# vocdoni/gnark-crypto-primitives

Measured on AMD Instinct MI355X. Metric: proofs/sec, Arbo-160 Poseidon SMT-verifier circuit, Groth16/BN254, higher is better.
Workload: dtype u32x8 Montgomery (254-bit integer)

## Files before the change

### gnark_crypto_primitives_amd/csrc/api.hip

```cpp
#include <algorithm>

#include "zkmi_internal.h"
#include "comb_plan.h"
#include "ff29.h"
#include "ec29.h"

using namespace zk;

namespace zk {

void sync_side_streams(zkmi_ctx* ctx) {
  for (hipStream_t q : {ctx->stream2, ctx->stream3, ctx->stream4})
    if (q) hipStreamSynchronize(q);
}

int ensure_scratch(zkmi_ctx* ctx, DevBuf& s, size_t bytes, void** out) {
  if (s.bytes < bytes) {
    if (s.p) {
      hipStreamSynchronize(ctx->stream);
      sync_side_streams(ctx);
      hipFree(s.p);
      s.p = nullptr;
      s.bytes = 0;
    }
// ... 334 lines not shown
  hipSetDevice(ctx->device);
  hipStreamSynchronize(ctx->stream);
  sync_side_streams(ctx);
  for (auto& st : ctx->sets) {
    if (st.ev0) hipEventDestroy(st.ev0);
    if (st.ev1) hipEventDestroy(st.ev1);
    for (auto& e : st.evq)
      if (e) hipEventDestroy(e);
    for (auto& e : st.eva)
      if (e) hipEventDestroy(e);
    if (st.tail_ev) hipEventDestroy(st.tail_ev);
    for (auto& p : st.msm_ev) {
      if (p[0]) hipEventDestroy(p[0]);
      if (p[1]) hipEventDestroy(p[1]);
    }
  }
  hipStreamDestroy(ctx->stream2);
  hipStreamDestroy(ctx->stream3);
  hipStreamDestroy(ctx->stream4);
  for (auto& p : ctx->plans) free_plan(p);
  for (auto& st : ctx->sets)
    for (DevBuf* b : {&st.slots, &st.a, &st.b, &st.c, &st.misc, &st.sums, &st.commit})
      if (b->p) hipFree(b->p);
  for (DevBuf* b : {&ctx->ntt_tmp, &ctx->build_tmp, &ctx->msm_digits, &ctx->msm_sint,
                    &ctx->msm_rowvar, &ctx->msm_part[0], &ctx->msm_part[1], &ctx->side_part2, &ctx->side_part3})
    if (b->p) hipFree(b->p);
  witness_ring_free(ctx);
  for (auto& e : ctx->ev)
    if (e) hipEventDestroy(e);
  for (auto& e : ctx->part_ev)
    if (e) hipEventDestroy(e);
  for (auto& e : ctx->acc_ev)
    if (e) hipEventDestroy(e);
  for (auto& e : ctx->dig_ev)
    if (e) hipEventDestroy(e);
  hipStreamDestroy(ctx->stream);
  delete ctx;
}

const char* zkmi_last_error(zkmi_ctx* ctx) { return ctx ? ctx->err.c_str() : "null context"; }

int zkmi_sync(zkmi_ctx* ctx) {
  ZK_HIP(hipStreamSynchronize(ctx->stream));
  return ZKMI_OK;
}

void* zkmi_stream(zkmi_ctx* ctx) { return (void*)ctx->stream; }
// ... 159 lines not shown
      if (plan.comb <= 8) return rc;
      plan = plan_comb(plan.comb - 1, plan.comb_signed != 0);
    } else if (plan.shared) {
      if (plan.bits[0] <= 4) return rc;
      plan = plan_shared(plan.bits[0] - 1);
    } else {
      if (plan.W >= 64) return rc;
      plan = plan_with_windows(plan.W + 1);
    }
  }
}

static bool window_bits_ok(int wb) {
  return wb == 0 || (wb >= 2 && wb <= 16) || (wb >= 104 && wb <= 116) ||
         (wb >= 202 && wb <= 220) || (wb >= 303 && wb <= 321);
}
static WinPlan plan_explicit(int wb) {
  return wb >= 300   ? plan_comb(wb - 300, true)
         : wb >= 200 ? plan_comb(wb - 200, false)
         : wb >= 100 ? plan_shared(wb - 100)
                     : plan_uniform(wb);
}
static double prove_working_set_bytes(uint32_t log_n, size_t n_slots, size_t n_in, size_t max_batch,
                                      size_t n_msm_max, size_t n_commitments) {
  const size_t Bp = round_up(max_batch ? max_batch : 1024, 64);
  const size_t n = (size_t)1 << log_n;
  const SetBytes sb = prove_set_bytes(n_slots, n, n_in, Bp, Bp);
  const double set = (double)(sb.slots + 3 * sb.abc + sb.misc + sums_bytes(Bp) +
                              commit_buffer_bytes(n_commitments, Bp));
  const double digits = 254.0 * (double)((n_msm_max + 15) / 16) * Bp * 4;
  const double sint = (double)n_msm_max * Bp * 32;
  const double partials = 2 * (21.0 * 254 * Bp * 256 + 256.0 * (double)((n_msm_max + 15) / 16) * 4);
  const double ring = 3.0 * std::max(68e6, (double)n_in * 32 * 64);
  return 2 * set + (double)n * Bp * 32 + digits + sint + partials + ring + 2e9 + 1e9;
}
static double free_hbm_bytes() {
  size_t free_b = 0, total_b = 0;
  if (hipMemGetInfo(&free_b, &total_b) != hipSuccess) free_b = (size_t)64 << 30;
  return (double)free_b;
}
static double usable_table_bytes_standalone(size_t n) {
  const double ws = (double)n * 1024 * 32 * 2 + 254.0 * ((n + 15) / 16) * 1024 * 4 +
                    21.0 * 254 * 1024 * 256 + 3e9;
  const double usable = free_hbm_bytes() - ws;
  return usable > 0 ? usable : 0.0;
}

int zkmi_msm_bases_load(zkmi_ctx* ctx, int group, const void* bases, size_t n, int window_bits,
                        zkmi_msm_bases** out) {
  return zkmi_msm_bases_load_image(ctx, group, bases, n, window_bits, 0, out);
}

int zkmi_msm_bases_load_image(zkmi_ctx* ctx, int group, const void* bases, size_t n,
                              int window_bits, int image, zkmi_msm_bases** out) {
  ZK_HIP(hipSetDevice(ctx->device));
  if (!out) return ZKMI_ERR_ARG;
  if (image != 0 && image != 1) {
// ... 301 lines not shown
  const uint32_t n_kb = fold.folded ? (uint32_t)fold.k_wire.size() : d->n_k;
  const uint32_t n_zb = fold.folded ? n_z + 1 : n_z;
  auto* pk = new zkmi_pk();
  pk->log_n = d->log_n;
  pk->n_wires = d->n_wires;
  pk->n_a = d->n_a;
  pk->n_b = d->n_b;
  pk->n_k = n_kb;
  pk->n_z = n_zb;
  pk->folded = fold.folded;
  pk->fold_n_constraints = fold.folded ? d->fold_r1cs->n_constraints : 0;
  pk->max_batch = d->max_batch ? d->max_batch : 1024;
  int rc;
  if ((rc = commit_keys_load(ctx, d, pk))) {
    zkmi_pk_free(ctx, pk);
    return rc;
  }
  const bool auto1 = d->window_bits_g1 == 0, auto2 = d->window_bits_g2 == 0;
  const size_t n1 = (size_t)d->n_a + d->n_b + n_kb + n_zb;
  const size_t n_msm_max = std::max(std::max((size_t)d->n_a, (size_t)d->n_b),
                                    std::max((size_t)n_kb, (size_t)n_zb));
  const size_t n_slots = d->n_slots_hint ? d->n_slots_hint : (size_t)d->n_wires + d->n_wires / 20;
  const double ws = prove_working_set_bytes(d->log_n, n_slots, d->n_wires, pk->max_batch, n_msm_max,
                                            pk->commits.size());
  double usable = free_hbm_bytes() - ws;
  if (usable < 0) usable = 0;
  if (d->table_budget_bytes && (double)d->table_budget_bytes < usable)
    usable = (double)d->table_budget_bytes;
  int sc1 = 0, sc2 = 0;
  plan_shared_for_budget(n1, d->n_b, 0.98 * usable, &sc1, &sc2);
  WinPlan p1 = auto1 ? plan_windows_for_budget(n1, 1, 0.64 * usable)
                     : plan_explicit((int)d->window_bits_g1);
  WinPlan p2 = auto2 ? plan_windows_for_budget(d->n_b, 2, 0.34 * usable)
                     : plan_explicit((int)d->window_bits_g2);
  if (auto1 && sc1 && plan_shared(sc1).W < p1.W) p1 = plan_shared(sc1);
  if (auto2 && sc2 && plan_shared(sc2).W < p2.W) p2 = plan_shared(sc2);
  WinPlan pm[COMB_PLAN_MSMS] = {p1, p1, p1, p1, p2};
  if (n1 >= 4096) {
    const size_t nm[COMB_PLAN_MSMS] = {auto1 ? d->n_a : 0u, auto1 ? d->n_b : 0u, auto1 ? n_kb : 0u,
                                       auto1 ? n_zb : 0u, auto2 ? d->n_b : 0u};
    const CombPlan eq = comb_plan_equal5(nm, 0.98 * usable, d->sparse_witness == 0);
    const CombPlan cp = comb_plan_search(nm, 0.98 * usable, d->sparse_witness == 0);
    for (int i = 0; i < COMB_PLAN_MSMS; i++) {
      const bool g2 = comb_msm_is_g2(i);
      if ((g2 ? auto2 : auto1) && (double)COMB_W / eq.k[i] < (double)(g2 ? p2 : p1).W)
        pm[i] = plan_comb(cp.k[i], cp.sg[i]);
    }
// ... 15 lines not shown
  bool relax[COMB_PLAN_MSMS] = {auto1, auto1, auto1, auto1, auto2};
  if (msm_window_bits)
    for (int i = 0; i < COMB_PLAN_MSMS; i++) {
      pm[i] = plan_explicit((int)msm_window_bits[i]);
      relax[i] = false;
    }
  auto load = [&](int group, const void* pts, size_t n, const WinPlan& plan, bool relax,
                  zkmi_msm_bases** out, int image) -> int {
    Staged sb(ctx);
    int r = sb.in(pts, n * (group == 1 ? 64 : 128));
    if (r) return r;
    r = bases_load_plan(ctx, group, sb.dev, n, plan, relax, out, image);
    if (!r) (*out)->chunk_factor = d->msm_chunk_factor;
    return r;
  };
  if ((rc = upload_u32(ctx, wa.data(), d->n_a, &pk->a_wire)) ||
      (rc = upload_u32(ctx, wb.data(), d->n_b, &pk->b_wire)) ||
      (rc = upload_u32(ctx, fold.folded ? fold.k_wire.data() : wk.data(), n_kb, &pk->k_wire)) ||
      (rc = load(1, d->g1_a, d->n_a, pm[COMB_MSM_A], relax[COMB_MSM_A], &pk->A, MSM_IMAGE_F)) ||
      (rc = load(1, d->g1_b, d->n_b, pm[COMB_MSM_B1], relax[COMB_MSM_B1], &pk->B1, MSM_IMAGE_F)) ||
      (rc = load(1, fold.folded ? (const void*)fold.k.data() : d->g1_k, n_kb, pm[COMB_MSM_K],
                 relax[COMB_MSM_K], &pk->K, MSM_IMAGE_F)) ||
      (rc = load(1, fold.folded ? (const void*)fold.e.data() : d->g1_z, n_zb, pm[COMB_MSM_Z],
                 relax[COMB_MSM_Z], &pk->Z, MSM_IMAGE_STD)) ||
      (rc = load(2, d->g2_b, d->n_b, pm[COMB_MSM_B2], relax[COMB_MSM_B2], &pk->B2, MSM_IMAGE_F))) {
    zkmi_pk_free(ctx, pk);
    return rc;
  }
  {
    const uint32_t idx[3] = {0, 1, 2};
    if ((rc = upload_u32(ctx, idx, 3, &pk->idx3)) ||
        (rc = zkmi_msm_bases_load(ctx, 1, d->g1_delta, 1, 8, &pk->D1)) ||
        (rc = zkmi_msm_bases_load(ctx, 2, d->g2_delta, 1, 8, &pk->D2))) {
      zkmi_pk_free(ctx, pk);
      return rc;
    }
    pk->D1->side = pk->D2->side = 2;
  }
  hipMemcpy(&pk->alpha, d->g1_alpha, 64, hipMemcpyDefault);
  hipMemcpy(&pk->beta1, d->g1_beta, 64, hipMemcpyDefault);
  hipMemcpy(&pk->delta1, d->g1_delta, 64, hipMemcpyDefault);
  hipMemcpy(&pk->beta2, d->g2_beta, 128, hipMemcpyDefault);
  hipMemcpy(&pk->delta2, d->g2_delta, 128, hipMemcpyDefault);
  *out = pk;
  return ZKMI_OK;
}

// ... 195 lines not shown
    if (!rc) rc = solve_rows(ctx, cs, slots, a, b, c, st, Bp, begin, cs->n_rows);
    if (!rc) rc = commit_finish_submit(ctx, S);
  }
  return prove_set_end(ctx, main, rc);
}

static int enqueue_heavy(zkmi_ctx* ctx, int si) {
  zkmi_ctx::ProveSet& S = ctx->sets[si];
  const zkmi_pk* pk = S.pk;
  const bool fd = S.f_domain;
  const size_t Bp = S.Bp, batch = S.batch, n = (size_t)1 << pk->log_n;
  NttPlan* plan;
  int rc = get_plan(ctx, (int)pk->log_n, &plan);
  if (rc) return rc;
  void* t0;
  if ((rc = ensure_scratch(ctx, ctx->ntt_tmp, n * Bp * 32, &t0))) return rc;
  SumsView v(S.sums.p, Bp);
  Fr* rs_bi = (Fr*)S.rs;
  Fr* slots = (Fr*)S.slots.p;
  ZK_HIP(hipStreamWaitEvent(ctx->stream, S.ev1, 0));
  hipEventRecord(S.evq[0], ctx->stream);
  Fr* h;
  if ((rc = pk->folded ? compute_ab_coset_bi(ctx, plan, (Fr*)S.a.p, (Fr*)S.b.p, (Fr*)t0, Bp,
                                             S.n_constraints, &h, fd)
                       : compute_h_bi(ctx, plan, (Fr*)S.a.p, (Fr*)S.b.p, (Fr*)S.c.p, (Fr*)t0, Bp,
                                      S.n_constraints, &h, fd)))
    return rc;
  hipEventRecord(S.evq[1], ctx->stream);
  S.msm_ev_used = 0;
  ctx->msm_ev_set = si;
  const bool d1 = pk->Z->plan.shared || pk->Z->plan.comb;
  const bool d2 = pk->B2->plan.shared || pk->B2->plan.comb;
  hipStream_t q3 = ctx->stream3, q4 = ctx->stream4;
  uint8_t* rv = nullptr;
  if (pk->A->plan.comb || pk->B2->plan.comb) {
    void* p;
    if ((rc = ensure_scratch(ctx, ctx->msm_rowvar, pk->n_wires, &p)) ||
        (rc = msm_rows_vary(ctx, slots, pk->n_wires, Bp, batch, (uint8_t*)p))) {
      ctx->msm_ev_set = -1;
      return rc;
    }
    rv = (uint8_t*)p;
  }
  if ((rc = msm_run(ctx, pk->A, slots, pk->a_wire, Bp, batch, v.sA, fd, d1 ? v.w1[0] : nullptr, q4,
                    rv)) ||
      (rc = msm_run(ctx, pk->B1, slots, pk->b_wire, Bp, batch, v.sB1, fd, d1 ? v.w1[1] : nullptr, q4,
                    rv)) ||
      (rc = msm_run(ctx, pk->K, slots, pk->k_wire, Bp, batch, v.sK, fd, d1 ? v.w1[2] : nullptr, q4,
                    rv)) ||
      (rc = msm_run(ctx, pk->Z, h, nullptr, Bp, batch, v.sZ, false, d1 ? v.w1[3] : nullptr, q4,
                    nullptr, true))) {
    ctx->msm_ev_set = -1;
    return rc;
  }
  hipEventRecord(S.evq[2], ctx->stream);
  rc = msm_run(ctx, pk->B2, slots, pk->b_wire, Bp, batch, v.sB2, fd, d2 ? v.w2 : nullptr, q4, rv);
  ctx->msm_ev_set = -1;
  if (rc) return rc;
  hipEventRecord(S.evq[3], ctx->stream);
  ZK_HIP(hipEventRecord(S.tail_ev, q4));
  {
    hipStream_t main_stream = ctx->stream;
    ZK_HIP(hipStreamWaitEvent(q3, S.ev1, 0));
    ctx->stream = q3;
    hipLaunchKernelGGL(rs_prep_kernel, dim3((unsigned)(Bp / 64)), dim3(64), 0, q3, rs_bi, Bp);
    (void)((rc = msm_run(ctx, pk->D1, rs_bi, pk->idx3 + 0, Bp, batch, v.tR)) ||
           (rc = msm_run(ctx, pk->D1, rs_bi, pk->idx3 + 1, Bp, batch, v.tS)) ||
           (rc = msm_run(ctx, pk->D1, rs_bi, pk->idx3 + 2, Bp, batch, v.tNRS)) ||
           (rc = msm_run(ctx, pk->D2, rs_bi, pk->idx3 + 1, Bp, batch, v.tS2)));
    ctx->stream = main_stream;
    if (rc) return rc;
  }
  if ((rc = commit_pok(ctx, S))) return rc;
  hipEventRecord(S.evq[4], ctx->stream);
// ... 109 lines not shown
```

### gnark_crypto_primitives_amd/csrc/ntt.hip

```cpp
#include <cstdlib>

#include "zkmi_internal.h"
#include "ff29.h"
#if defined(__HIP_DEVICE_COMPILE__)
#include "ff29_asm.h"
#endif

namespace zk {

__device__ __forceinline__ uint32_t pass_row(uint32_t hi, uint32_t q, uint32_t lo, int s0, int K) {
  return (hi << (s0 + K)) | (q << s0) | lo;
}

__device__ __forceinline__ uint32_t bitrev32(uint32_t x, int bits) {
  return __brev(x) >> (32 - bits);
}

__device__ __forceinline__ Fr29 ld29(const Fr* base, size_t row, size_t b, size_t Bp) {
  const Fr v = bi_ld(base, row, b, Bp);
  return unpack29<Fr29Params>(v.v);
}
__device__ __forceinline__ Fr29 ldz29(const Fr* base, size_t row, size_t b, size_t Bp) {
  const Fr v = bi_ld(base, row, b, Bp);
  return unpack_lazy<Fr29Params>(v.v);
}
__device__ __forceinline__ Fr29 ldc29(const Fr* tab, uint32_t i) {
  return unpack29<Fr29Params>(tab[i].v);
}

template <class T> __device__ __forceinline__ T ld_tw(const Fr* tw, uint32_t i);
template <> __device__ __forceinline__ Fr ld_tw<Fr>(const Fr* tw, uint32_t i) { return tw[i]; }
template <> __device__ __forceinline__ Fr29 ld_tw<Fr29>(const Fr* tw, uint32_t i) {
  return ldc29(tw, i);
}
__device__ __forceinline__ Fr tmul(const Fr& a, const Fr& tw) { return mul(a, tw); }
#if defined(__HIP_DEVICE_COMPILE__)
__device__ __forceinline__ Fr29 tmul(const Fr29& a, const Fr29& tw) { return mul_asm_s(a, tw); }
#else
ZK_HD Fr29 tmul(const Fr29& a, const Fr29& tw) { return mul(a, tw); }
#endif

template <int J0, int NJ, int LQ = J0, bool FROM0 = false, class T, int M>
__device__ __forceinline__ void butterflies(T (&x)[M], uint32_t qb, int log_n, int s0, uint32_t lo,
                                            const Fr* __restrict__ tw) {
#pragma unroll
  for (int j = J0; j < J0 + NJ; j++) {
    const int s = (FROM0 ? 0 : s0) + j, jj = j - LQ;
// ... 126 lines not shown
#pragma unroll
  for (int i = 0; i < 4; i++) {
    const uint32_t q = w + 4 * i;
    const uint4 l = xch[(q * 2 + 0) * 64 + lane], h = xch[(q * 2 + 1) * 64 + lane];
    x[i].v[0] = l.x; x[i].v[1] = l.y; x[i].v[2] = l.z; x[i].v[3] = l.w;
    x[i].v[4] = h.x; x[i].v[5] = h.y; x[i].v[6] = h.z; x[i].v[7] = h.w;
  }
  butterflies<2, 2, 2, FIRST>(x, w, log_n, s0, lo, tw);
#pragma unroll
  for (int i = 0; i < 4; i++)
    store_scaled<LAST>(dst, pass_row(hi, w + 4 * i, lo, s0, 4), b, Bp, x[i], post, post_uniform,
                       use_uniform);
}

template <bool FIRST, bool LAST>
__global__ __launch_bounds__(256) void ntt_pass4_lds29(const Fr* __restrict__ src,
                                                       Fr* __restrict__ dst, size_t Bp, int log_n,
                                                       int s0, const Fr* __restrict__ tw,
                                                       const Fr* __restrict__ pre, int in_std,
                                                       const Fr* __restrict__ post,
                                                       Fr post_uniform, int use_uniform,
                                                       uint32_t n_valid,
                                                       const Fr* __restrict__ sub_after,
                                                       const Fr* __restrict__ times) {
  __shared__ int32_t xch[16 * 9 * 64];
  const uint32_t lane = threadIdx.x;
  const size_t b = (size_t)blockIdx.x * 64 + lane;
  const uint32_t w = __builtin_amdgcn_readfirstlane(threadIdx.y);
  const uint32_t g = blockIdx.y;
  const uint32_t lo = g & ((1u << s0) - 1u);
  const uint32_t hi = g >> s0;
  Fr29 x[4];
#pragma unroll
  for (int i = 0; i < 4; i++) {
    const uint32_t row = pass_row(hi, 4 * w + i, lo, s0, 4);
    x[i] = FIRST ? first_load29(src, row, b, Bp, log_n, n_valid, pre, in_std)
                 : ldz29(dst, row, b, Bp);
  }
  butterflies<0, 2, 0, FIRST>(x, 4 * w, log_n, s0, lo, tw);
  exchange29(xch, x, w, w, lane);
  butterflies<2, 2, 2, FIRST>(x, w, log_n, s0, lo, tw);
#pragma unroll
  for (int i = 0; i < 4; i++) {
    const uint32_t row = pass_row(hi, w + 4 * i, lo, s0, 4);
    Fr out;
    if (LAST && (use_uniform || post)) {
      const Fr29 k = use_uniform ? unpack29<Fr29Params>(post_uniform.v) : ldc29(post, row);
      Fr29 v = norm(x[i]);
      if (times) v = mul(v, ldz29(times, row, b, Bp));
      pack_canonical<Fr29Params>(out.v, mul(v, k));
      if (sub_after) out = sub(out, bi_ld(sub_after, row, b, Bp));
    } else {
      pack_lazy<Fr29Params>(out.v, wred(x[i]));
    }
    bi_st(dst, row, b, Bp, out);
  }
}

template <int K>
__global__ __launch_bounds__(256) void ntt_mid29(Fr* __restrict__ dst, size_t Bp, int log_n, int s0,
                                                 const Fr* __restrict__ tw) {
  const size_t b = (size_t)blockIdx.x * 64 + threadIdx.x;
  const uint32_t g =
      __builtin_amdgcn_readfirstlane(blockIdx.y * blockDim.y + threadIdx.y);
  const uint32_t lo = g & ((1u << s0) - 1u);
  const uint32_t hi = g >> s0;
  constexpr int M = 1 << K;
  Fr29 x[M];
#pragma unroll
  for (int i = 0; i < M; i++) x[i] = ldz29(dst, pass_row(hi, i, lo, s0, K), b, Bp);
  butterflies<0, (K < 2 ? K : 2)>(x, 0, log_n, s0, lo, tw);
  if constexpr (K == 3) {
#pragma unroll
    for (int i = 0; i < M; i++) x[i] = norm(x[i]);
    butterflies<2, 1, 0>(x, 0, log_n, s0, lo, tw);
  }
#pragma unroll
  for (int i = 0; i < M; i++) {
    Fr out;
    pack_lazy<Fr29Params>(out.v, wred(x[i]));
    bi_st(dst, pass_row(hi, i, lo, s0, K), b, Bp, out);
  }
}

template <bool PRODUCT>
__global__ __launch_bounds__(256) void ntt_fused29(const Fr* __restrict__ src,
                                                   Fr* __restrict__ dst, size_t Bp, int log_n,
                                                   const Fr* __restrict__ tw_last,
                                                   const Fr* __restrict__ tw_first,
                                                   const Fr* __restrict__ factor) {
  __shared__ int32_t xch[16 * 9 * 64];
  const uint32_t lane = threadIdx.x;
  const size_t b = (size_t)blockIdx.x * 64 + lane;
  const uint32_t w = __builtin_amdgcn_readfirstlane(threadIdx.y);
  const int s0 = log_n - 4;
  const uint32_t lo = blockIdx.y;
  Fr29 x[4];
#pragma unroll
  for (int i = 0; i < 4; i++) x[i] = ldz29(src, pass_row(0, 4 * w + i, lo, s0, 4), b, Bp);
  butterflies<0, 2>(x, 4 * w, log_n, s0, lo, tw_last);
  exchange29(xch, x, w, w, lane);
  butterflies<2, 2>(x, w, log_n, s0, lo, tw_last);
  Fr29 y[4];
#pragma unroll
  for (int i = 0; i < 4; i++) {
    const uint32_t row = pass_row(0, w + 4 * i, lo, s0, 4);
    y[i] = mul(norm(x[i]), PRODUCT ? ldz29(factor, row, b, Bp) : ldc29(factor, row));
  }
  const uint32_t wp = ((w & 1u) << 1) | (w >> 1);
  x[0] = y[0];
  x[1] = y[2];
  x[2] = y[1];
  x[3] = y[3];
  butterflies<0, 2, 0, true>(x, 4 * wp, log_n, 0, 0, tw_first);
  __syncthreads();
  exchange29(xch, x, wp, w, lane);
  butterflies<2, 2, 2, true>(x, w, log_n, 0, 0, tw_first);
  const uint32_t hi = bitrev32(lo, s0);
#pragma unroll
  for (int i = 0; i < 4; i++) {
    Fr out;
    pack_lazy<Fr29Params>(out.v, wred(x[i]));
    bi_st(dst, pass_row(hi, w + 4 * i, 0, 0, 4), b, Bp, out);
  }
}

__global__ __launch_bounds__(256) void pointwise_h_kernel(const Fr* __restrict__ a,
                                                          const Fr* __restrict__ b,
                                                          const Fr* __restrict__ c,
                                                          Fr* __restrict__ h, size_t total,
                                                          size_t Bp, Fr den) {
  size_t i = (size_t)blockIdx.x * blockDim.x + threadIdx.x;
  const size_t stride = (size_t)gridDim.x * blockDim.x;
  for (; i < total; i += stride) {
    const size_t row = i / Bp, l = i % Bp;
    Fr t = sub(mul(bi_ld(a, row, l, Bp), bi_ld(b, row, l, Bp)), bi_ld(c, row, l, Bp));
    bi_st(h, row, l, Bp, mul(t, den));
  }
}


__global__ __launch_bounds__(256) void transpose_in_kernel(const uint4* __restrict__ src,
                                                           uint4* __restrict__ dst, size_t rows,
                                                           size_t batch, size_t Bp, int q16) {
  size_t total = rows * Bp * q16;
  size_t i = (size_t)blockIdx.x * blockDim.x + threadIdx.x;
  const size_t stride = (size_t)gridDim.x * blockDim.x;
// ... 130 lines not shown
  }
  for (size_t i = 0; i < n; i++) {
    cf29[i] = mul(cf[i], k261);
    cf29n[i] = mul(cf29[i], p.n_inv);
  }
  p.ninv_den = mul(p.n_inv, p.den);
  int rc;
  if ((rc = upload(ctx, &p.tw_fwd, twf)) || (rc = upload(ctx, &p.tw_inv, twi)) ||
      (rc = upload(ctx, &p.coset_fwd, cf)) || (rc = upload(ctx, &p.coset_inv, ci)) ||
      (rc = upload(ctx, &p.coset_inv_den, cid)) ||
      (rc = upload(ctx, &p.tw29_fwd, twf29)) || (rc = upload(ctx, &p.tw29_inv, twi29)) ||
      (rc = upload(ctx, &p.coset29_fwd, cf29)) || (rc = upload(ctx, &p.coset29n_fwd, cf29n))) {
    free_plan(p);
    return rc;
  }
  ctx->plans.push_back(p);
  *out = &ctx->plans.back();
  return ZKMI_OK;
}

typedef void (*PassFn)(const Fr*, Fr*, size_t, int, int, const Fr*, const Fr*, const Fr*, Fr, int,
                       uint32_t);
typedef void (*Pass29Fn)(const Fr*, Fr*, size_t, int, int, const Fr*, const Fr*, int, const Fr*,
                         Fr, int, uint32_t, const Fr*, const Fr*);
typedef void (*Mid29Fn)(Fr*, size_t, int, int, const Fr*);

static PassFn pick_pass(int k, bool first, bool last) {
  static const PassFn fn[3][2][2] = {
      {{ntt_pass<1, false, false>, ntt_pass<1, false, true>},
       {ntt_pass<1, true, false>, ntt_pass<1, true, true>}},
      {{ntt_pass<2, false, false>, ntt_pass<2, false, true>},
       {ntt_pass<2, true, false>, ntt_pass<2, true, true>}},
      {{ntt_pass4_lds<false, false>, ntt_pass4_lds<false, true>},
       {ntt_pass4_lds<true, false>, ntt_pass4_lds<true, true>}}};
  return fn[k == 4 ? 2 : k - 1][first][last];
}
static Pass29Fn pick_pass29(bool first, bool last) {
  static const Pass29Fn fn[2][2] = {{ntt_pass4_lds29<false, false>, ntt_pass4_lds29<false, true>},
                                    {ntt_pass4_lds29<true, false>, ntt_pass4_lds29<true, true>}};
  return fn[first][last];
}
static Mid29Fn pick_mid29(int k) {
  static const Mid29Fn fn[3] = {ntt_mid29<1>, ntt_mid29<2>, ntt_mid29<3>};
  return fn[k - 1];
}

struct Post29 {
  const Fr* table = nullptr;
  Fr factor = Fr::zero();
  int use_factor = 0;
  const Fr* sub_after = nullptr;
  const Fr* times = nullptr;
  static Post29 none() { return Post29(); }
  static Post29 uniform(const Fr& k) {
    Post29 p;
    p.factor = k;
    p.use_factor = 1;
    return p;
  }
  static Post29 per_row(const Fr* table, const Fr* sub_after = nullptr) {
    Post29 p;
    p.table = table;
    p.sub_after = sub_after;
    return p;
  }
  static Post29 times_rows(const Fr* m, const Fr& k) {
    Post29 p = uniform(k);
    p.times = m;
    return p;
  }
};
enum Image29 { IN_F = 0, IN_STD = 1 };

static int ntt29(zkmi_ctx* ctx, const NttPlan* plan, const Fr* src, Fr* dst, size_t Bp,
                 const Fr* tw, Image29 in, const Fr* pre, size_t n_valid, const Post29& post,
                 int s_from, int s_to) {
  const int log_n = plan->log_n, rem = log_n % 4;
  const dim3 block(64, 4);
  for (int s0 = s_from; s0 < s_to;) {
    if (rem && s0 == 4) {
      const Mid29Fn mid = pick_mid29(rem);
      hipLaunchKernelGGL(mid, dim3((unsigned)(Bp / 64), 1u << (log_n - rem - 2)), block, 0,
                         ctx->stream, dst, Bp, log_n, s0, tw);
      s0 += rem;
      continue;
    }
    const Pass29Fn pass = pick_pass29(s0 == 0, s0 + 4 == log_n);
    hipLaunchKernelGGL(pass, dim3((unsigned)(Bp / 64), 1u << (log_n - 4)), block, 0, ctx->stream,
                       src, dst, Bp, log_n, s0, tw, pre, (int)in, post.table, post.factor,
                       post.use_factor, (uint32_t)n_valid, post.sub_after, post.times);
    s0 += 4;
  }
  ZK_HIP(hipGetLastError());
  return ZKMI_OK;
}

int ntt_bi(zkmi_ctx* ctx, const NttPlan* plan, const Fr* src, Fr* dst, size_t Bp, bool inverse,
           bool coset, size_t n_valid) {
  const int log_n = plan->log_n;
  if (log_n >= 8 && src != dst) {
    const Post29 post = (inverse && coset) ? Post29::per_row(plan->coset_inv)
                                           : Post29::uniform(inverse ? plan->n_inv : Fr::one());
    return ntt29(ctx, plan, src, dst, Bp, inverse ? plan->tw29_inv : plan->tw29_fwd, IN_STD,
                 (!inverse && coset) ? plan->coset29_fwd : nullptr, n_valid, post, 0, log_n);
  }
  const Fr* tw = inverse ? plan->tw_inv : plan->tw_fwd;
  const Fr* pre = (!inverse && coset) ? plan->coset_fwd : nullptr;
  const Fr* post = (inverse && coset) ? plan->coset_inv : nullptr;
  const int use_uniform = (inverse && !coset) ? 1 : 0;
  for (int s0 = 0, k; s0 < log_n; s0 += k) {
    k = (log_n - s0) % 4;
    k = k == 0 ? 4 : k > 2 ? 2 : k;
    const uint32_t groups = 1u << (log_n - k);
    const uint32_t waves = (k == 4 || groups >= 4) ? 4 : groups;
    const dim3 block(64, waves), grid((unsigned)(Bp / 64), k == 4 ? groups : groups / waves);
    const PassFn pass = pick_pass(k, s0 == 0, s0 + k == log_n);
    hipLaunchKernelGGL(pass, grid, block, 0, ctx->stream, src, dst, Bp, log_n, s0, tw, pre, post,
                       plan->n_inv, use_uniform, (uint32_t)n_valid);
  }
  ZK_HIP(hipGetLastError());
  return ZKMI_OK;
}

static int pointwise_h(zkmi_ctx* ctx, const NttPlan* plan, const Fr* a, const Fr* b, const Fr* c,
                       Fr* h, size_t Bp) {
  const size_t total = ((size_t)1 << plan->log_n) * Bp;
  hipLaunchKernelGGL(pointwise_h_kernel, dim3(grid_for(total, 256)), dim3(256), 0, ctx->stream, a,
                     b, c, h, total, Bp, plan->den);
  ZK_HIP(hipGetLastError());
  return ZKMI_OK;
}

static int to_coset29(zkmi_ctx* ctx, const NttPlan* plan, Fr* x, Fr* t0, size_t Bp, size_t n_valid,
                      Image29 in, int s_to, const Post29& post) {
  const int lg = plan->log_n;
  const Fr *inv = plan->tw29_inv, *fwd = plan->tw29_fwd;
  int rc;
  if ((rc = ntt29(ctx, plan, x, t0, Bp, inv, in, nullptr, n_valid, Post29::none(), 0, lg - 4)))
    return rc;
  hipLaunchKernelGGL(ntt_fused29<false>, dim3((unsigned)(Bp / 64), 1u << (lg - 4)), dim3(64, 4), 0,
                     ctx->stream, t0, x, Bp, lg, inv, fwd, plan->coset29n_fwd);
  return ntt29(ctx, plan, x, x, Bp, fwd, IN_F, nullptr, (size_t)1 << lg, post, 4, s_to);
}

int compute_h_bi(zkmi_ctx* ctx, const NttPlan* plan, Fr* a, Fr* b, Fr* c, Fr* t0, size_t Bp,
                 size_t n_valid, Fr** h_out, bool abc_f) {
  const int lg = plan->log_n;
  const size_t n = (size_t)1 << lg;
  int rc;
  if (lg < 8) {
    for (Fr* x : {a, b, c}) {
      if (abc_f && (rc = rows_to_std_domain(ctx, x, n_valid, Bp))) return rc;
      if ((rc = ntt_bi(ctx, plan, x, t0, Bp, true, false, n_valid))) return rc;
      if ((rc = ntt_bi(ctx, plan, t0, x, Bp, false, true, n))) return rc;
    }
    if ((rc = pointwise_h(ctx, plan, a, b, c, a, Bp))) return rc;
    if ((rc = ntt_bi(ctx, plan, a, t0, Bp, true, true, n))) return rc;
    *h_out = t0;
    return ZKMI_OK;
  }
  const Image29 in = abc_f ? IN_F : IN_STD;
  const Fr *inv = plan->tw29_inv, *fwd = plan->tw29_fwd;
  const dim3 fgrid((unsigned)(Bp / 64), 1u << (lg - 4)), fblock(64, 4);
  if ((rc = to_coset29(ctx, plan, a, t0, Bp, n_valid, in, lg, Post29::none())) ||
      (rc = to_coset29(ctx, plan, b, t0, Bp, n_valid, in, lg - 4, Post29::none())))
    return rc;
  hipLaunchKernelGGL(ntt_fused29<true>, fgrid, fblock, 0, ctx->stream, b, t0, Bp, lg, fwd, inv, a);
  if ((rc = ntt29(ctx, plan, c, b, Bp, inv, in, nullptr, n_valid, Post29::uniform(plan->ninv_den),
                  0, lg)))
    return rc;
  if ((rc = ntt29(ctx, plan, t0, t0, Bp, inv, IN_F, nullptr, n,
                  Post29::per_row(plan->coset_inv_den, b), 4, lg)))
    return rc;
  *h_out = t0;
  return ZKMI_OK;
}

int compute_ab_coset_bi(zkmi_ctx* ctx, const NttPlan* plan, Fr* a, Fr* b, Fr* t0, size_t Bp,
                        size_t n_valid, Fr** u_out, bool abc_f) {
  const int lg = plan->log_n;
  if (lg < 8) {
    ctx->err = "compute_ab_coset_bi: domains below 2^8 keep compute_h_bi";
    return ZKMI_ERR_ARG;
  }
  const Image29 in = abc_f ? IN_F : IN_STD;
  int rc;
  if ((rc = to_coset29(ctx, plan, a, t0, Bp, n_valid, in, lg, Post29::none())) ||
      (rc = to_coset29(ctx, plan, b, t0, Bp, n_valid, in, lg, Post29::times_rows(a, Fr::one()))))
    return rc;
  *u_out = b;
  return ZKMI_OK;
}

}
```

### gnark_crypto_primitives_amd/csrc/zkmi_internal.h

```cpp
#pragma once
#include <hip/hip_runtime.h>
#include <stdint.h>
#include <string>
#include <utility>
#include <vector>

#include "../../include/zkmi.h"
#include "ec.h"
#include "vprog.h"

namespace zk {


struct DevBuf {
  void* p = nullptr;
  size_t bytes = 0;
};

struct NttPlan {
  int log_n = 0;
  Fr* tw_fwd = nullptr;
  Fr* tw_inv = nullptr;
  Fr* coset_fwd = nullptr;
  Fr* coset_inv = nullptr;
  Fr* coset_inv_den = nullptr;
  Fr n_inv;
  Fr den;
  Fr ninv_den;
  Fr* tw29_fwd = nullptr;
  Fr* tw29_inv = nullptr;
  Fr* coset29_fwd = nullptr;
  Fr* coset29n_fwd = nullptr;
};

}

struct zkmi_ctx {
  int device = 0;
  hipStream_t stream = nullptr;
  std::string err;
  std::vector<zk::NttPlan> plans;
  hipEvent_t ev[8] = {};
  double timings[8] = {};
  zk::DevBuf ntt_tmp;
  zk::DevBuf build_tmp;
  zk::DevBuf msm_digits, msm_sint;
  zk::DevBuf msm_rowvar;
  zk::DevBuf msm_part[2];
  zk::DevBuf side_part2;
  zk::DevBuf side_part3;
  hipStream_t stream2 = nullptr, stream3 = nullptr, stream4 = nullptr;
  struct ProveSet {
    bool pending = false;
    bool heavy_enqueued = false;
    zk::DevBuf slots, a, b, c, misc, sums, commit;
    hipEvent_t evq[5] = {};
    hipEvent_t eva[2] = {};
    hipEvent_t tail_ev = nullptr;
    hipEvent_t msm_ev[8][2] = {};
    int msm_ev_group[8] = {};
    int msm_ev_used = 0;
    size_t batch = 0, Bp = 0;
    const zkmi_pk* pk = nullptr;
    const zkmi_cs* cs = nullptr;
    size_t n_constraints = 0;
    bool f_domain = true;
    void *rs = nullptr, *st = nullptr;
// ... 177 lines not shown
  ~Staged() {
    if (owned && dev) {
      hipStreamSynchronize(ctx->stream);
      hipFree(dev);
    }
  }
};
int device_view(zkmi_ctx* ctx, const void* src, size_t bytes, void* stage, const void** out);

int prove_set_begin(zkmi_ctx* ctx, const zkmi_pk* pk, size_t value_rows, size_t n_staged,
                    size_t batch, const void* rs, hipStream_t* main, char** stage);
int prove_set_end(zkmi_ctx* ctx, hipStream_t main, int rc);

int transpose_in(zkmi_ctx* ctx, const void* src_pm, void* dst_bi, size_t rows, size_t batch,
                 size_t Bp, size_t elem_bytes);
int transpose_out(zkmi_ctx* ctx, const void* src_bi, void* dst_pm, size_t rows, size_t batch,
                  size_t Bp, size_t elem_bytes);

int get_plan(zkmi_ctx* ctx, int log_n, NttPlan** out);
void free_plan(NttPlan& p);
int ntt_bi(zkmi_ctx* ctx, const NttPlan* plan, const Fr* src, Fr* dst, size_t Bp, bool inverse,
           bool coset, size_t n_valid);
int compute_h_bi(zkmi_ctx* ctx, const NttPlan* plan, Fr* a, Fr* b, Fr* c, Fr* t0, size_t Bp,
                 size_t n_valid, Fr** h_out, bool abc_f = false);

int compute_ab_coset_bi(zkmi_ctx* ctx, const NttPlan* plan, Fr* a, Fr* b, Fr* t0, size_t Bp,
                        size_t n_valid, Fr** u_out, bool abc_f = false);

struct FoldedKey {
  bool folded = false;
  std::vector<G1Affine> e, k;
  std::vector<uint32_t> k_wire;
};
int quotient_fold_key(zkmi_ctx* ctx, const zkmi_pk_desc* d, const std::vector<uint32_t>& k_wire,
                      FoldedKey* out);
int quotient_bases_dev(zkmi_ctx* ctx, const NttPlan* plan, const G1Affine* z_dev, uint32_t n_z,
                       G1Affine* pts);

constexpr int COMB_W = 254;
constexpr uint32_t COMB_MIN_GROUPS_PER_CHUNK = 32;
WinPlan plan_with_windows(int W);
WinPlan plan_uniform(int c);
WinPlan plan_shared(int c);
WinPlan plan_comb(int k, bool signed_tables = true);
WinPlan plan_windows_for_budget(size_t n_total, int group, double budget_bytes);
void plan_comb_for_budget(size_t n1, size_t n2, double usable_bytes, int* k1, int* k2, bool* sg1,
                          bool* sg2, bool allow_signed = true);
void plan_shared_for_budget(size_t n1, size_t n2, double usable_bytes, int* c1, int* c2);
enum { MSM_IMAGE_STD = 0, MSM_IMAGE_F = 1 };
int msm_bases_build(zkmi_ctx* ctx, int group, const void* bases_dev, size_t n, const WinPlan& plan,
// ... 30 lines not shown
```

Baseline: 9033.

## Store NTT intermediates as raw 29-bit limbs with a separate top-limb plane

Intermediate NTT passes now write the 29-bit limb representation directly: eight low limbs go into the Fr buffer and the ninth limb goes into a new int32 plane, instead of packing and unpacking lazily at every pass. This removes pack/unpack and weak-reduction arithmetic between passes, at the cost of an extra 4 bytes per element of memory traffic and extra scratch allocation, which is also added to the working-set estimate. For the folded path, the quotient output stays in Montgomery form (out_f) and the Z MSM loads F-image bases, which skips a conversion.

```diff
diff --git a/gnark_crypto_primitives_amd/csrc/api.hip b/gnark_crypto_primitives_amd/csrc/api.hip
--- a/gnark_crypto_primitives_amd/csrc/api.hip
+++ b/gnark_crypto_primitives_amd/csrc/api.hip
@@ -380,7 +380,7 @@
   for (auto& st : ctx->sets)
     for (DevBuf* b : {&st.slots, &st.a, &st.b, &st.c, &st.misc, &st.sums, &st.commit})
       if (b->p) hipFree(b->p);
-  for (DevBuf* b : {&ctx->ntt_tmp, &ctx->build_tmp, &ctx->msm_digits, &ctx->msm_sint,
+  for (DevBuf* b : {&ctx->ntt_tmp, &ctx->ntt_top, &ctx->build_tmp, &ctx->msm_digits, &ctx->msm_sint,
                     &ctx->msm_rowvar, &ctx->msm_part[0], &ctx->msm_part[1], &ctx->side_part2, &ctx->side_part3})
     if (b->p) hipFree(b->p);
   witness_ring_free(ctx);
@@ -586,7 +586,7 @@
                      : plan_uniform(wb);
 }
 static double prove_working_set_bytes(uint32_t log_n, size_t n_slots, size_t n_in, size_t max_batch,
-                                      size_t n_msm_max, size_t n_commitments) {
+                                      size_t n_msm_max, size_t n_commitments, bool folded) {
   const size_t Bp = round_up(max_batch ? max_batch : 1024, 64);
   const size_t n = (size_t)1 << log_n;
   const SetBytes sb = prove_set_bytes(n_slots, n, n_in, Bp, Bp);
@@ -596,7 +596,8 @@
   const double sint = (double)n_msm_max * Bp * 32;
   const double partials = 2 * (21.0 * 254 * Bp * 256 + 256.0 * (double)((n_msm_max + 15) / 16) * 4);
   const double ring = 3.0 * std::max(68e6, (double)n_in * 32 * 64);
-  return 2 * set + (double)n * Bp * 32 + digits + sint + partials + ring + 2e9 + 1e9;
+  const double planes = (folded || log_n < 8) ? 0.0 : 3.0 * (double)n * Bp * 4;
+  return 2 * set + (double)n * Bp * 32 + planes + digits + sint + partials + ring + 2e9 + 1e9;
 }
 static double free_hbm_bytes() {
   size_t free_b = 0, total_b = 0;
@@ -944,7 +945,7 @@
                                     std::max((size_t)n_kb, (size_t)n_zb));
   const size_t n_slots = d->n_slots_hint ? d->n_slots_hint : (size_t)d->n_wires + d->n_wires / 20;
   const double ws = prove_working_set_bytes(d->log_n, n_slots, d->n_wires, pk->max_batch, n_msm_max,
-                                            pk->commits.size());
+                                            pk->commits.size(), pk->folded);
   double usable = free_hbm_bytes() - ws;
   if (usable < 0) usable = 0;
   if (d->table_budget_bytes && (double)d->table_budget_bytes < usable)
@@ -1006,7 +1007,7 @@
       (rc = load(1, fold.folded ? (const void*)fold.k.data() : d->g1_k, n_kb, pm[COMB_MSM_K],
                  relax[COMB_MSM_K], &pk->K, MSM_IMAGE_F)) ||
       (rc = load(1, fold.folded ? (const void*)fold.e.data() : d->g1_z, n_zb, pm[COMB_MSM_Z],
-                 relax[COMB_MSM_Z], &pk->Z, MSM_IMAGE_STD)) ||
+                 relax[COMB_MSM_Z], &pk->Z, fold.folded ? MSM_IMAGE_F : MSM_IMAGE_STD)) ||
       (rc = load(2, d->g2_b, d->n_b, pm[COMB_MSM_B2], relax[COMB_MSM_B2], &pk->B2, MSM_IMAGE_F))) {
     zkmi_pk_free(ctx, pk);
     return rc;
@@ -1248,7 +1249,7 @@
   hipEventRecord(S.evq[0], ctx->stream);
   Fr* h;
   if ((rc = pk->folded ? compute_ab_coset_bi(ctx, plan, (Fr*)S.a.p, (Fr*)S.b.p, (Fr*)t0, Bp,
-                                             S.n_constraints, &h, fd)
+                                             S.n_constraints, &h, fd, (int32_t*)S.c.p, true)
                        : compute_h_bi(ctx, plan, (Fr*)S.a.p, (Fr*)S.b.p, (Fr*)S.c.p, (Fr*)t0, Bp,
                                       S.n_constraints, &h, fd)))
     return rc;
@@ -1274,8 +1275,8 @@
                     rv)) ||
       (rc = msm_run(ctx, pk->K, slots, pk->k_wire, Bp, batch, v.sK, fd, d1 ? v.w1[2] : nullptr, q4,
                     rv)) ||
-      (rc = msm_run(ctx, pk->Z, h, nullptr, Bp, batch, v.sZ, false, d1 ? v.w1[3] : nullptr, q4,
-                    nullptr, true))) {
+      (rc = msm_run(ctx, pk->Z, h, nullptr, Bp, batch, v.sZ, pk->folded, d1 ? v.w1[3] : nullptr,
+                    q4, nullptr, true))) {
     ctx->msm_ev_set = -1;
     return rc;
   }
diff --git a/gnark_crypto_primitives_amd/csrc/ntt.hip b/gnark_crypto_primitives_amd/csrc/ntt.hip
--- a/gnark_crypto_primitives_amd/csrc/ntt.hip
+++ b/gnark_crypto_primitives_amd/csrc/ntt.hip
@@ -20,9 +20,30 @@
   const Fr v = bi_ld(base, row, b, Bp);
   return unpack29<Fr29Params>(v.v);
 }
-__device__ __forceinline__ Fr29 ldz29(const Fr* base, size_t row, size_t b, size_t Bp) {
+__device__ __forceinline__ Fr29 ldraw29(const Fr* base, const int32_t* top, size_t row, size_t b,
+                                        size_t Bp) {
   const Fr v = bi_ld(base, row, b, Bp);
-  return unpack_lazy<Fr29Params>(v.v);
+  Fr29 r;
+#pragma unroll
+  for (int l = 0; l < 8; l++) r.v[l] = (int32_t)v.v[l];
+  r.v[8] = top[row * Bp + b];
+  return r;
+}
+__device__ __forceinline__ Fr29 ldl29(const Fr* base, const int32_t* top, size_t row, size_t b,
+                                      size_t Bp) {
+  return norm(ldraw29(base, top, row, b, Bp));
+}
+__device__ __forceinline__ Fr29 ldw29(const Fr* base, const int32_t* top, size_t row, size_t b,
+                                      size_t Bp) {
+  return wred(ldraw29(base, top, row, b, Bp));
+}
+__device__ __forceinline__ void stl29(Fr* base, int32_t* top, size_t row, size_t b, size_t Bp,
+                                      const Fr29& x) {
+  Fr w;
+#pragma unroll
+  for (int l = 0; l < 8; l++) w.v[l] = (uint32_t)x.v[l];
+  bi_st(base, row, b, Bp, w);
+  top[row * Bp + b] = x.v[8];
 }
 __device__ __forceinline__ Fr29 ldc29(const Fr* tab, uint32_t i) {
   return unpack29<Fr29Params>(tab[i].v);
@@ -195,7 +216,9 @@
                                                        Fr post_uniform, int use_uniform,
                                                        uint32_t n_valid,
                                                        const Fr* __restrict__ sub_after,
-                                                       const Fr* __restrict__ times) {
+                                                       const Fr* __restrict__ times,
+                                                       int32_t* __restrict__ dst_top,
+                                                       const int32_t* __restrict__ times_top) {
   __shared__ int32_t xch[16 * 9 * 64];
   const uint32_t lane = threadIdx.x;
   const size_t b = (size_t)blockIdx.x * 64 + lane;
@@ -208,7 +231,7 @@
   for (int i = 0; i < 4; i++) {
     const uint32_t row = pass_row(hi, 4 * w + i, lo, s0, 4);
     x[i] = FIRST ? first_load29(src, row, b, Bp, log_n, n_valid, pre, in_std)
-                 : ldz29(dst, row, b, Bp);
+                 : ldl29(dst, dst_top, row, b, Bp);
   }
   butterflies<0, 2, 0, FIRST>(x, 4 * w, log_n, s0, lo, tw);
   exchange29(xch, x, w, w, lane);
@@ -216,22 +239,25 @@
 #pragma unroll
   for (int i = 0; i < 4; i++) {
     const uint32_t row = pass_row(hi, w + 4 * i, lo, s0, 4);
-    Fr out;
-    if (LAST && (use_uniform || post)) {
-      const Fr29 k = use_uniform ? unpack29<Fr29Params>(post_uniform.v) : ldc29(post, row);
+    if (LAST && (use_uniform || post || times)) {
+      Fr out;
       Fr29 v = norm(x[i]);
-      if (times) v = mul(v, ldz29(times, row, b, Bp));
-      pack_canonical<Fr29Params>(out.v, mul(v, k));
+      if (times) v = mul(v, ldw29(times, times_top, row, b, Bp));
+      if (use_uniform || post)
+        v = mul(v, use_uniform ? unpack29<Fr29Params>(post_uniform.v) : ldc29(post, row));
+      pack_canonical<Fr29Params>(out.v, v);
       if (sub_after) out = sub(out, bi_ld(sub_after, row, b, Bp));
+      bi_st(dst, row, b, Bp, out);
     } else {
-      pack_lazy<Fr29Params>(out.v, wred(x[i]));
+      stl29(dst, dst_top, row, b, Bp, x[i]);
     }
-    bi_st(dst, row, b, Bp, out);
   }
 }
 
 template <int K>
-__global__ __launch_bounds__(256) void ntt_mid29(Fr* __restrict__ dst, size_t Bp, int log_n, int s0,
+__global__ __launch_bounds__(256) void ntt_mid29(Fr* __restrict__ dst,
+                                                 int32_t* __restrict__ dst_top, size_t Bp,
+                                                 int log_n, int s0,
                                                  const Fr* __restrict__ tw) {
   const size_t b = (size_t)blockIdx.x * 64 + threadIdx.x;
   const uint32_t g =
@@ -241,7 +267,7 @@
   constexpr int M = 1 << K;
   Fr29 x[M];
 #pragma unroll
-  for (int i = 0; i < M; i++) x[i] = ldz29(dst, pass_row(hi, i, lo, s0, K), b, Bp);
+  for (int i = 0; i < M; i++) x[i] = ldl29(dst, dst_top, pass_row(hi, i, lo, s0, K), b, Bp);
   butterflies<0, (K < 2 ? K : 2)>(x, 0, log_n, s0, lo, tw);
   if constexpr (K == 3) {
 #pragma unroll
@@ -249,11 +275,7 @@
     butterflies<2, 1, 0>(x, 0, log_n, s0, lo, tw);
   }
 #pragma unroll
-  for (int i = 0; i < M; i++) {
-    Fr out;
-    pack_lazy<Fr29Params>(out.v, wred(x[i]));
-    bi_st(dst, pass_row(hi, i, lo, s0, K), b, Bp, out);
-  }
+  for (int i = 0; i < M; i++) stl29(dst, dst_top, pass_row(hi, i, lo, s0, K), b, Bp, x[i]);
 }
 
 template <bool PRODUCT>
@@ -261,7 +283,10 @@
                                                    Fr* __restrict__ dst, size_t Bp, int log_n,
                                                    const Fr* __restrict__ tw_last,
                                                    const Fr* __restrict__ tw_first,
-                                                   const Fr* __restrict__ factor) {
+                                                   const Fr* __restrict__ factor,
+                                                   const int32_t* __restrict__ src_top,
+                                                   int32_t* __restrict__ dst_top,
+                                                   const int32_t* __restrict__ factor_top) {
   __shared__ int32_t xch[16 * 9 * 64];
   const uint32_t lane = threadIdx.x;
   const size_t b = (size_t)blockIdx.x * 64 + lane;
@@ -270,7 +295,8 @@
   const uint32_t lo = blockIdx.y;
   Fr29 x[4];
 #pragma unroll
-  for (int i = 0; i < 4; i++) x[i] = ldz29(src, pass_row(0, 4 * w + i, lo, s0, 4), b, Bp);
+  for (int i = 0; i < 4; i++)
+    x[i] = ldl29(src, src_top, pass_row(0, 4 * w + i, lo, s0, 4), b, Bp);
   butterflies<0, 2>(x, 4 * w, log_n, s0, lo, tw_last);
   exchange29(xch, x, w, w, lane);
   butterflies<2, 2>(x, w, log_n, s0, lo, tw_last);
@@ -278,7 +304,8 @@
 #pragma unroll
   for (int i = 0; i < 4; i++) {
     const uint32_t row = pass_row(0, w + 4 * i, lo, s0, 4);
-    y[i] = mul(norm(x[i]), PRODUCT ? ldz29(factor, row, b, Bp) : ldc29(factor, row));
+    y[i] = mul(norm(x[i]),
+               PRODUCT ? ldw29(factor, factor_top, row, b, Bp) : ldc29(factor, row));
   }
   const uint32_t wp = ((w & 1u) << 1) | (w >> 1);
   x[0] = y[0];
@@ -291,11 +318,7 @@
   butterflies<2, 2, 2, true>(x, w, log_n, 0, 0, tw_first);
   const uint32_t hi = bitrev32(lo, s0);
 #pragma unroll
-  for (int i = 0; i < 4; i++) {
-    Fr out;
-    pack_lazy<Fr29Params>(out.v, wred(x[i]));
-    bi_st(dst, pass_row(hi, w + 4 * i, 0, 0, 4), b, Bp, out);
-  }
+  for (int i = 0; i < 4; i++) stl29(dst, dst_top, pass_row(hi, w + 4 * i, 0, 0, 4), b, Bp, x[i]);
 }
 
 __global__ __launch_bounds__(256) void pointwise_h_kernel(const Fr* __restrict__ a,
@@ -472,8 +495,8 @@
 typedef void (*PassFn)(const Fr*, Fr*, size_t, int, int, const Fr*, const Fr*, const Fr*, Fr, int,
                        uint32_t);
 typedef void (*Pass29Fn)(const Fr*, Fr*, size_t, int, int, const Fr*, const Fr*, int, const Fr*,
-                         Fr, int, uint32_t, const Fr*, const Fr*);
-typedef void (*Mid29Fn)(Fr*, size_t, int, int, const Fr*);
+                         Fr, int, uint32_t, const Fr*, const Fr*, int32_t*, const int32_t*);
+typedef void (*Mid29Fn)(Fr*, int32_t*, size_t, int, int, const Fr*);
 
 static PassFn pick_pass(int k, bool first, bool last) {
   static const PassFn fn[3][2][2] = {
@@ -501,6 +524,7 @@
   int use_factor = 0;
   const Fr* sub_after = nullptr;
   const Fr* times = nullptr;
+  const int32_t* times_top = nullptr;
   static Post29 none() { return Post29(); }
   static Post29 uniform(const Fr& k) {
     Post29 p;
@@ -514,35 +538,50 @@
     p.sub_after = sub_after;
     return p;
   }
-  static Post29 times_rows(const Fr* m, const Fr& k) {
+  static Post29 times_rows(const Fr* m, const int32_t* m_top, const Fr& k) {
     Post29 p = uniform(k);
     p.times = m;
+    p.times_top = m_top;
+    return p;
+  }
+  static Post29 times_rows(const Fr* m, const int32_t* m_top) {
+    Post29 p;
+    p.times = m;
+    p.times_top = m_top;
     return p;
   }
 };
 enum Image29 { IN_F = 0, IN_STD = 1 };
 
-static int ntt29(zkmi_ctx* ctx, const NttPlan* plan, const Fr* src, Fr* dst, size_t Bp,
-                 const Fr* tw, Image29 in, const Fr* pre, size_t n_valid, const Post29& post,
-                 int s_from, int s_to) {
+static int ntt29(zkmi_ctx* ctx, const NttPlan* plan, const Fr* src, Fr* dst, int32_t* dst_top,
+                 size_t Bp, const Fr* tw, Image29 in, const Fr* pre, size_t n_valid,
+                 const Post29& post, int s_from, int s_to) {
   const int log_n = plan->log_n, rem = log_n % 4;
   const dim3 block(64, 4);
   for (int s0 = s_from; s0 < s_to;) {
     if (rem && s0 == 4) {
       const Mid29Fn mid = pick_mid29(rem);
       hipLaunchKernelGGL(mid, dim3((unsigned)(Bp / 64), 1u << (log_n - rem - 2)), block, 0,
-                         ctx->stream, dst, Bp, log_n, s0, tw);
+                         ctx->stream, dst, dst_top, Bp, log_n, s0, tw);
       s0 += rem;
       continue;
     }
     const Pass29Fn pass = pick_pass29(s0 == 0, s0 + 4 == log_n);
     hipLaunchKernelGGL(pass, dim3((unsigned)(Bp / 64), 1u << (log_n - 4)), block, 0, ctx->stream,
                        src, dst, Bp, log_n, s0, tw, pre, (int)in, post.table, post.factor,
-                       post.use_factor, (uint32_t)n_valid, post.sub_after, post.times);
+                       post.use_factor, (uint32_t)n_valid, post.sub_after, post.times, dst_top,
+                       post.times_top);
     s0 += 4;
   }
   ZK_HIP(hipGetLastError());
   return ZKMI_OK;
+}
+
+static int limb_planes(zkmi_ctx* ctx, const NttPlan* plan, size_t Bp, int count, int32_t** out) {
+  void* p;
+  const int rc = ensure_scratch(ctx, ctx->ntt_top, ((size_t)count << plan->log_n) * Bp * 4, &p);
+  *out = (int32_t*)p;
+  return rc;
 }
 
 int ntt_bi(zkmi_ctx* ctx, const NttPlan* plan, const Fr* src, Fr* dst, size_t Bp, bool inverse,
@@ -551,7 +590,9 @@
   if (log_n >= 8 && src != dst) {
     const Post29 post = (inverse && coset) ? Post29::per_row(plan->coset_inv)
                                            : Post29::uniform(inverse ? plan->n_inv : Fr::one());
-    return ntt29(ctx, plan, src, dst, Bp, inverse ? plan->tw29_inv : plan->tw29_fwd, IN_STD,
+    int32_t* top;
+    if (int rc = limb_planes(ctx, plan, Bp, 1, &top)) return rc;
+    return ntt29(ctx, plan, src, dst, top, Bp, inverse ? plan->tw29_inv : plan->tw29_fwd, IN_STD,
                  (!inverse && coset) ? plan->coset29_fwd : nullptr, n_valid, post, 0, log_n);
   }
   const Fr* tw = inverse ? plan->tw_inv : plan->tw_fwd;
@@ -581,20 +622,23 @@
   return ZKMI_OK;
 }
 
-static int to_coset29(zkmi_ctx* ctx, const NttPlan* plan, Fr* x, Fr* t0, size_t Bp, size_t n_valid,
-                      Image29 in, int s_to, const Post29& post) {
+static int to_coset29(zkmi_ctx* ctx, const NttPlan* plan, Fr* x, int32_t* x_top, Fr* t0,
+                      int32_t* t0_top, size_t Bp, size_t n_valid, Image29 in, int s_to,
+                      const Post29& post) {
   const int lg = plan->log_n;
   const Fr *inv = plan->tw29_inv, *fwd = plan->tw29_fwd;
   int rc;
-  if ((rc = ntt29(ctx, plan, x, t0, Bp, inv, in, nullptr, n_valid, Post29::none(), 0, lg - 4)))
+  if ((rc = ntt29(ctx, plan, x, t0, t0_top, Bp, inv, in, nullptr, n_valid, Post29::none(), 0,
+                  lg - 4)))
     return rc;
   hipLaunchKernelGGL(ntt_fused29<false>, dim3((unsigned)(Bp / 64), 1u << (lg - 4)), dim3(64, 4), 0,
-                     ctx->stream, t0, x, Bp, lg, inv, fwd, plan->coset29n_fwd);
-  return ntt29(ctx, plan, x, x, Bp, fwd, IN_F, nullptr, (size_t)1 << lg, post, 4, s_to);
+                     ctx->stream, t0, x, Bp, lg, inv, fwd, plan->coset29n_fwd, t0_top, x_top,
+                     (const int32_t*)nullptr);
+  return ntt29(ctx, plan, x, x, x_top, Bp, fwd, IN_F, nullptr, (size_t)1 << lg, post, 4, s_to);
 }
 
 int compute_h_bi(zkmi_ctx* ctx, const NttPlan* plan, Fr* a, Fr* b, Fr* c, Fr* t0, size_t Bp,
-                 size_t n_valid, Fr** h_out, bool abc_f) {
+                 size_t n_valid, Fr** h_out, bool abc_f, int32_t* top) {
   const int lg = plan->log_n;
   const size_t n = (size_t)1 << lg;
   int rc;
@@ -612,14 +656,17 @@
   const Image29 in = abc_f ? IN_F : IN_STD;
   const Fr *inv = plan->tw29_inv, *fwd = plan->tw29_fwd;
   const dim3 fgrid((unsigned)(Bp / 64), 1u << (lg - 4)), fblock(64, 4);
-  if ((rc = to_coset29(ctx, plan, a, t0, Bp, n_valid, in, lg, Post29::none())) ||
-      (rc = to_coset29(ctx, plan, b, t0, Bp, n_valid, in, lg - 4, Post29::none())))
+  if (!top && (rc = limb_planes(ctx, plan, Bp, 3, &top))) return rc;
+  int32_t *a_top = top, *b_top = top + n * Bp, *t0_top = top + 2 * n * Bp;
+  if ((rc = to_coset29(ctx, plan, a, a_top, t0, t0_top, Bp, n_valid, in, lg, Post29::none())) ||
+      (rc = to_coset29(ctx, plan, b, b_top, t0, t0_top, Bp, n_valid, in, lg - 4, Post29::none())))
     return rc;
-  hipLaunchKernelGGL(ntt_fused29<true>, fgrid, fblock, 0, ctx->stream, b, t0, Bp, lg, fwd, inv, a);
-  if ((rc = ntt29(ctx, plan, c, b, Bp, inv, in, nullptr, n_valid, Post29::uniform(plan->ninv_den),
-                  0, lg)))
+  hipLaunchKernelGGL(ntt_fused29<true>, fgrid, fblock, 0, ctx->stream, b, t0, Bp, lg, fwd, inv, a,
+                     b_top, t0_top, a_top);
+  if ((rc = ntt29(ctx, plan, c, b, b_top, Bp, inv, in, nullptr, n_valid,
+                  Post29::uniform(plan->ninv_den), 0, lg)))
     return rc;
-  if ((rc = ntt29(ctx, plan, t0, t0, Bp, inv, IN_F, nullptr, n,
+  if ((rc = ntt29(ctx, plan, t0, t0, t0_top, Bp, inv, IN_F, nullptr, n,
                   Post29::per_row(plan->coset_inv_den, b), 4, lg)))
     return rc;
   *h_out = t0;
@@ -627,16 +674,21 @@
 }
 
 int compute_ab_coset_bi(zkmi_ctx* ctx, const NttPlan* plan, Fr* a, Fr* b, Fr* t0, size_t Bp,
-                        size_t n_valid, Fr** u_out, bool abc_f) {
+                        size_t n_valid, Fr** u_out, bool abc_f, int32_t* top, bool out_f) {
   const int lg = plan->log_n;
   if (lg < 8) {
     ctx->err = "compute_ab_coset_bi: domains below 2^8 keep compute_h_bi";
     return ZKMI_ERR_ARG;
   }
   const Image29 in = abc_f ? IN_F : IN_STD;
+  const size_t n = (size_t)1 << lg;
   int rc;
-  if ((rc = to_coset29(ctx, plan, a, t0, Bp, n_valid, in, lg, Post29::none())) ||
-      (rc = to_coset29(ctx, plan, b, t0, Bp, n_valid, in, lg, Post29::times_rows(a, Fr::one()))))
+  if (!top && (rc = limb_planes(ctx, plan, Bp, 3, &top))) return rc;
+  int32_t *a_top = top, *b_top = top + n * Bp, *t0_top = top + 2 * n * Bp;
+  if ((rc = to_coset29(ctx, plan, a, a_top, t0, t0_top, Bp, n_valid, in, lg, Post29::none())) ||
+      (rc = to_coset29(ctx, plan, b, b_top, t0, t0_top, Bp, n_valid, in, lg,
+                       out_f ? Post29::times_rows(a, a_top)
+                             : Post29::times_rows(a, a_top, Fr::one()))))
     return rc;
   *u_out = b;
   return ZKMI_OK;
diff --git a/gnark_crypto_primitives_amd/csrc/zkmi_internal.h b/gnark_crypto_primitives_amd/csrc/zkmi_internal.h
--- a/gnark_crypto_primitives_amd/csrc/zkmi_internal.h
+++ b/gnark_crypto_primitives_amd/csrc/zkmi_internal.h
@@ -43,6 +43,7 @@
   hipEvent_t ev[8] = {};
   double timings[8] = {};
   zk::DevBuf ntt_tmp;
+  zk::DevBuf ntt_top;
   zk::DevBuf build_tmp;
   zk::DevBuf msm_digits, msm_sint;
   zk::DevBuf msm_rowvar;
@@ -266,10 +267,11 @@
 int ntt_bi(zkmi_ctx* ctx, const NttPlan* plan, const Fr* src, Fr* dst, size_t Bp, bool inverse,
            bool coset, size_t n_valid);
 int compute_h_bi(zkmi_ctx* ctx, const NttPlan* plan, Fr* a, Fr* b, Fr* c, Fr* t0, size_t Bp,
-                 size_t n_valid, Fr** h_out, bool abc_f = false);
+                 size_t n_valid, Fr** h_out, bool abc_f = false, int32_t* top = nullptr);
 
 int compute_ab_coset_bi(zkmi_ctx* ctx, const NttPlan* plan, Fr* a, Fr* b, Fr* t0, size_t Bp,
-                        size_t n_valid, Fr** u_out, bool abc_f = false);
+                        size_t n_valid, Fr** u_out, bool abc_f = false, int32_t* top = nullptr,
+                        bool out_f = false);
 
 struct FoldedKey {
   bool folded = false;
```

Result: faster. 9155 (median of 6 runs) (+1.3%).
